# ut-vision/Rot-MVGaze

Hardware: AMD Instinct MI355X
Metric: multi-view samples/sec (fwd+bwd), BxVx3x224x224 (higher is better)
Workload: dtype f32; 1 GPU; C3: ResNet-50, V=4, B=128 per GPU, 3x224x224, fwd+loss+bwd; backbone=ResNet-50, views=4, batch_per_gpu=128, global_batch=128, image=3x224x224, parallelism=dp1, weights=random init, seed 0 (kaiming-normal convs, default Linear), rccl_ranks=1, step_launch=eager: every kernel queued from Python

## Files before the change

include/rotmvgaze.h:

```cpp
#ifndef ROTMVGAZE_H
#define ROTMVGAZE_H

#include <stddef.h>
#include <stdint.h>

#ifdef __cplusplus
extern "C" {
#endif

#define MVG_ABI_VERSION 13

int mvg_abi_version(void);
const char *mvg_last_error(void);
int mvg_device_cus(void);
int mvg_set_scratch(void *ptr, size_t bytes, void *stream);
size_t mvg_scratch_bytes(void);
void *mvg_stream_create_low_priority(void);
int mvg_set_reserved_cus(int n);

enum {
  MVG_K_CONV_FPROP = 0, MVG_K_CONV_DGRAD = 1, MVG_K_CONV_WGRAD = 2, MVG_K_WGRAD_REDUCE = 3,
  MVG_K_BN_FINALIZE = 4, MVG_K_BN_APPLY = 5, MVG_K_BN_BWD_REDUCE = 6, MVG_K_BN_BWD_APPLY = 7,
  MVG_K_POOL = 8, MVG_K_LAYOUT = 9, MVG_K_LINEAR_FPROP = 10, MVG_K_LINEAR_DGRAD = 11,
  MVG_K_LINEAR_WGRAD = 12, MVG_K_ROTCAT = 13, MVG_K_COLSUM = 14, MVG_K_LOSS = 15,
// ... 320 lines not shown
int mvg_bn_apply_split_scaled(const float *y, const float *scale, const float *shift, const void *residual, int residual_sp,
                              const float *res_scale, const float *res_shift, const float *res_sinv, int relu, void *out_sp,
                              const float *out_sinv, uint8_t *relu_bits, int groups, int64_t rows_per_group, int c,
                              void *stream);
int mvg_bn_relu_maxpool_fwd_split_scaled(const float *y, const float *scale, const float *shift, void *pooled_sp,
                                         const float *pooled_sinv, uint8_t *argmax, int groups, int n_per_group, int h, int w,
                                         int c, int ho, int wo, void *stream);
int mvg_avgpool_fwd_split_scaled(const void *x_sp, const float *x_sinv, float *y, int n, int hw, int c, void *stream);
int mvg_conv_dgrad_bn_partials_split(const mvg_conv_desc *d);
int mvg_conv_dgrad_split_bnreduce(const mvg_conv_desc *d, const void *dy_sp, const float *dy_sinv, const void *w_crsk_sp,
                                  const float *w_sinv, float *dx, const float *addend, const float *bn_y, const uint8_t *bn_bits,
                                  const float *bn_mean, const float *bn_invstd, const float *relu_scale, const float *relu_shift,
                                  float *partials, float *s1, float *s2, float *dgamma, float *dbeta, int accumulate,
                                  float *mx, const float *bn_gamma, float *dx_dy_sinv, void *stream);
int mvg_conv_dgrad_split_bnapply_bnreduce(const mvg_conv_desc *d, void *dy_sp, const float *dy_sinv, const float *dz, const float *y,
                                          const float *mean, const float *invstd, const float *gamma, const float *un_s1,
                                          const float *un_s2, int64_t rows_per_group, const void *w_crsk_sp, const float *w_sinv,
                                          float *dx, const float *addend, const float *bn_y, const uint8_t *bn_bits,
                                          const float *bn_mean, const float *bn_invstd, const float *relu_scale,
                                          const float *relu_shift, float *partials, float *s1, float *s2, float *dgamma, float *dbeta,
                                          int accumulate, float *mx, const float *bn_gamma, float *dx_dy_sinv, void *stream);
int mvg_conv_fprop_split_stages(const mvg_conv_desc *d);
int mvg_conv_dgrad_split_stages(const mvg_conv_desc *d, int fused_reduce);
int mvg_conv_fprop_split_bnapply(const mvg_conv_desc *d, void *out_sp, const float *out_sinv, const float *bn_y, const float *scale,
                                 const float *shift, const void *residual, int residual_sp, const float *res_scale,
                                 const float *res_shift, const float *res_sinv, uint8_t *relu_bits, const void *w_sp,
                                 const float *w_sinv, float *y, float *stats, void *stream);
int mvg_stem_rowwindow_split(const float *x_nhwc4, void *xw_sp, int64_t images, int h, int w, void *stream);
int mvg_stem_rowwindow_split_nchw(const float *x_nchw, void *xw_sp, int64_t images, int h, int w, void *stream);
int mvg_stem_fprop_split(const mvg_conv_desc *d, const void *xw_sp, const void *w_sp, const float *w_sinv, float *y, float *stats,
                         void *stream);
int mvg_stem_wgrad_splits_split(const mvg_conv_desc *d);
int mvg_stem_wgrad_split(const mvg_conv_desc *d, const void *xw_sp, const void *dy_sp, const float *dy_sinv, float *dw_rw,
                         float *workspace, int splits, int accumulate, void *stream);
int mvg_bn_relu_maxpool_bwd_reduce_split(const float *g_pooled, const uint8_t *argmax, const float *y, const float *mean,
                                         const float *invstd, const float *scale, const float *shift, int groups,
                                         int n_per_group, int h, int w, int c, int ho, int wo, float *s1, float *s2,
                                         float *dgamma, float *dbeta, int accumulate, float *workspace, float *mx, const float *gamma,
                                         float *dy_sinv, void *stream);
int mvg_bn_relu_maxpool_bwd_apply_split(const float *g_pooled, const uint8_t *argmax, const float *y, const float *mean,
                                        const float *invstd, const float *gamma, const float *scale, const float *shift,
                                        const float *s1, const float *s2, int groups, int n_per_group, int h, int w, int c,
                                        int ho, int wo, void *dy_sp, const float *mx, float *dy_sinv, int dy_sinv_ready, void *stream);
int mvg_conv_wgrad_splits_split(const mvg_conv_desc *d);
int mvg_conv_wgrad_split_tile(const mvg_conv_desc *d, int32_t *bm, int32_t *bn, int32_t *incremental);
int mvg_conv_wgrad_split(const mvg_conv_desc *d, const void *x_sp, const void *dy_sp, const float *dy_sinv, float *dw,
// ... 63 lines not shown
```

rot-mvgaze_amd/_lib.py:

```python
from __future__ import annotations

import ctypes as C
import os

_HERE = os.path.dirname(os.path.abspath(__file__))
LIB_PATH = os.path.join(_HERE, "csrc", "librotmvgaze_hip.so")

K_FAMILIES = 18
ABI_VERSION = 13
SESSION_FP32, SESSION_BF16 = 0, 1


class ConvDesc(C.Structure):
    _fields_ = [(n, C.c_int32) for n in
                ("groups", "n", "h", "w", "cin", "cout", "r", "s", "stride", "pad", "ho", "wo")]

    @classmethod
    def make(cls, groups, n, h, w, cin, cout, k, stride, pad):
        ho = (h + 2 * pad - k) // stride + 1
        wo = (w + 2 * pad - k) // stride + 1
        return cls(groups, n, h, w, cin, cout, k, k, stride, pad, ho, wo)

    @classmethod
    def linear(cls, rows, fin, fout):
# ... 81 lines not shown
    "mvg_bn_apply_split": (_I, [_P, _P, _P, _P, _I, _P, _P, _I, _P, _P, _I, _I64, _I, _P]),
    "mvg_bn_bwd_apply_split": (_I, [_P, _P, _P, _P, _P, _P, _P, _P, _P, _I, _I64, _I, _P, _P, _P, _I, _P]),
    "mvg_bn_bwd_reduce_split": (_I, [_P, _P, _P, _P, _P, _P, _P, _I, _I64, _I, _P, _P, _P, _P, _I, _P, _P, _P, _P, _P, _P]),
    "mvg_bn_relu_maxpool_fwd_split": (_I, [_P, _P, _P, _P, _P, _I, _I, _I, _I, _I, _I, _I, _P]),
    "mvg_avgpool_fwd_split": (_I, [_P, _P, _I, _I, _I, _P]),
    "mvg_act_scales": (_I, [_P, _I, _P, _I, _P]),
    "mvg_bn_apply_split_scaled": (_I, [_P, _P, _P, _P, _I, _P, _P, _P, _I, _P, _P, _P, _I, _I64, _I, _P]),
    "mvg_bn_relu_maxpool_fwd_split_scaled": (_I, [_P, _P, _P, _P, _P, _P, _I, _I, _I, _I, _I, _I, _I, _P]),
    "mvg_avgpool_fwd_split_scaled": (_I, [_P, _P, _P, _I, _I, _I, _P]),
    "mvg_conv_wgrad_split_xs": (_I, [_D, _P, _P, _P, _P, _P, _P, _I, _I, _P]),
    "mvg_conv_wgrad_split_slabs_xs": (_I, [_D, _P, _P, _P, _P, _P, _I, _P]),
    "mvg_stem_rowwindow_split": (_I, [_P, _P, _I64, _I, _I, _P]),
    "mvg_stem_rowwindow_split_nchw": (_I, [_P, _P, _I64, _I, _I, _P]),
    "mvg_stem_fprop_split": (_I, [_D, _P, _P, _P, _P, _P, _P]),
    "mvg_stem_wgrad_splits_split": (_I, [_D]),
    "mvg_stem_wgrad_split": (_I, [_D, _P, _P, _P, _P, _P, _I, _I, _P]),
    "mvg_bn_relu_maxpool_bwd_reduce_split": (_I, [_P, _P, _P, _P, _P, _P, _P, _I, _I, _I, _I, _I, _I, _I, _P, _P, _P, _P, _I, _P, _P, _P, _P, _P]),
    "mvg_bn_relu_maxpool_bwd_apply_split": (_I, [_P, _P, _P, _P, _P, _P, _P, _P, _P, _P, _I, _I, _I, _I, _I, _I, _I, _P, _P, _P, _I, _P]),
    "mvg_conv_dgrad_bn_partials_split": (_I, [_D]),
    "mvg_conv_dgrad_split_bnreduce": (_I, [_D, _P, _P, _P, _P, _P, _P, _P, _P, _P, _P, _P, _P, _P, _P, _P, _P, _P, _I, _P, _P, _P, _P]),
    "mvg_conv_dgrad_split_bnapply_bnreduce": (_I, [_D] + [_P] * 9 + [_I64] + [_P] * 15 + [_I, _P, _P, _P, _P]),
    "mvg_conv_fprop_split_stages": (_I, [_D]),
    "mvg_conv_dgrad_split_stages": (_I, [_D, _I]),
    "mvg_conv_fprop_split_bnapply": (_I, [_D] + [_P] * 6 + [_I] + [_P] * 9),
    "mvg_conv_wgrad_splits_split": (_I, [_D]),
    "mvg_conv_wgrad_split_tile": (_I, [_D, C.POINTER(C.c_int32), C.POINTER(C.c_int32), C.POINTER(C.c_int32)]),
    "mvg_conv_wgrad_split": (_I, [_D, _P, _P, _P, _P, _P, _I, _I, _P]),
    "mvg_conv_wgrad_split_slabs": (_I, [_D, _P, _P, _P, _P, _I, _P]),
    "mvg_wgrad_reduce_batch": (_I, [C.POINTER(C.c_void_p), C.POINTER(C.c_void_p), C.POINTER(C.c_int64), C.POINTER(C.c_int32),
                                    C.POINTER(C.c_int32), _I, _P]),
    "mvg_bn_apply_bits": (_I, [_P, _P, _P, _P, _P, _P, _P, _P, _I, _I64, _I, _P]),
    "mvg_bn_bwd_reduce_bits": (_I, [_P, _P, _P, _P, _P, _I, _I64, _I, _P, _P, _P, _P, _I, _P, _P, _P]),
    "mvg_bn_apply_bits_bf16": (_I, [_P, _P, _P, _P, _P, _P, _P, _P, _I, _I64, _I, _P]),
    "mvg_bn_bwd_reduce_bits_bf16": (_I, [_P, _P, _P, _P, _P, _I, _I64, _I, _P, _P, _P, _P, _I, _P, _P, _P]),
    "mvg_bn_bwd_workspace_floats": (C.c_size_t, [_I, _I64, _I]),
    "mvg_bn_bwd_apply": (_I, [_P, _P, _P, _P, _P, _P, _P, _P, _P, _P, _I, _I64, _I, _P, _P, _P]),
    "mvg_maxpool3x3s2_fwd": (_I, [_P, _P, _P, _I, _I, _I, _I, _I, _I, _P]),
    "mvg_maxpool3x3s2_bwd": (_I, [_P, _P, _P, _I, _I, _I, _I, _I, _I, _P]),
    "mvg_bn_relu_maxpool_fwd": (_I, [_P, _P, _P, _P, _P, _I, _I, _I, _I, _I, _I, _I, _P]),
    "mvg_bn_relu_maxpool_bwd_reduce": (_I, [_P, _P, _P, _P, _P, _P, _P, _I, _I, _I, _I, _I, _I, _I, _P, _P, _P, _P, _I, _P,
                                            _P]),
    "mvg_bn_relu_maxpool_bwd_apply": (_I, [_P, _P, _P, _P, _P, _P, _P, _P, _P, _P, _I, _I, _I, _I, _I, _I, _I, _P, _P]),
    "mvg_bn_eval_bwd": (_I, [_P, _P, _P, _P, _P, _P, _P, _P, _P, _F, _I, _I64, _I, _P, _P, _P, _P, _I, _P, _P]),
    "mvg_bn_eval_bwd_workspace_floats": (C.c_size_t, [_I, _I64, _I]),
    "mvg_bn_relu_maxpool_eval_bwd": (_I, [_P, _P, _P, _P, _P, _P, _P, _P, _F, _I, _I, _I, _I, _I, _I, _I, _P, _P, _P, _I, _P,
                                          _P]),
# ... 114 lines not shown
```

rot-mvgaze_amd/csrc/conv_split.hip:

```cpp
#include "bf16_tile.h"
#include "elem.h"

namespace mvg {

typedef _Float16 f16x8 __attribute__((ext_vector_type(8)));

#define SPLIT_ONE(PA, PB, av, bv, acc)                                                                         \
  _Pragma("unroll") for (int i = 0; i < TM; ++i) _Pragma("unroll") for (int j = 0; j < TN; ++j)                \
      acc[i][j] = __builtin_amdgcn_mfma_f32_32x32x16_f16(av[PA][i], bv[PB][j], acc[i][j], 0, 0, 0);
#define SPLIT_PRODUCTS(av, bv, acc) SPLIT_ONE(0, 1, av, bv, acc) SPLIT_ONE(1, 0, av, bv, acc) SPLIT_ONE(0, 0, av, bv, acc)

constexpr int SP_BM = 128, SP_BK = 32;

__global__ __launch_bounds__(256) void split_f32_kernel(const float4 *__restrict__ x, uint4 *__restrict__ out, long long n8, float scale) {
  const long long stride = (long long)gridDim.x * 256;
  for (long long i = (long long)blockIdx.x * 256 + threadIdx.x; i < n8; i += stride) {
    const float4 lo = x[2 * i], hi = x[2 * i + 1];
    const float v[8] = {lo.x * scale, lo.y * scale, lo.z * scale, lo.w * scale, hi.x * scale, hi.y * scale, hi.z * scale, hi.w * scale};
    uint4 q1, q2;
    split2_chunk(v, q1, q2);
    out[2 * i] = q1;
    out[2 * i + 1] = q2;
  }
}
// ... 308 lines not shown
    if constexpr (AFFINE) {
      unpack8(rv[i], r);
    } else {
      const uint4 r1 = make_uint4(__float_as_uint(rv[i][0].x), __float_as_uint(rv[i][0].y), __float_as_uint(rv[i][0].z), __float_as_uint(rv[i][0].w));
      const uint4 r2 = make_uint4(__float_as_uint(rv[i][1].x), __float_as_uint(rv[i][1].y), __float_as_uint(rv[i][1].z), __float_as_uint(rv[i][1].w));
      merge2_chunk(r1, r2, r);
    }
    mb[i] = bn_apply_chunk(v, sc, sh, true, r, AFFINE, rs, rh, !AFFINE, rsi, true, osc, o);
#pragma unroll
    for (int k = 0; k < 8; ++k) o[k] = ok ? o[k] : 0.f;
  }
  __device__ __forceinline__ void store_extra(int i, unsigned off) {
    if (bits_out) bits_out[off >> 5] = (unsigned short)mb[i];
  }
};

#define MVG_SPLIT_RNG 0
#include "conv_split_igemm.inc"
#undef MVG_SPLIT_RNG
#define MVG_SPLIT_RNG 1
#include "conv_split_igemm.inc"
#undef MVG_SPLIT_RNG

template <int BM, int BN, bool INCR>
__global__ __launch_bounds__(256, BN >= 256 ? 2 : 3) void wgrad_split_kernel(WgradParams p) {
  constexpr int BK = 16, WGM = 2, WGN = 2;
  constexpr int WTM = BM / WGM, WTN = BN / WGN;
  constexpr int TM = WTM / 32, TN = WTN / 32;
  constexpr int LDA = BM + 32, LDB = BN + 32;
  constexpr int MV = BM / 8, NVB = BN / 8;
  constexpr int A_TPR = 256 / BK;
  constexpr int A_CPT = MV / A_TPR > 0 ? MV / A_TPR : 1;
  constexpr int B_CPT = (NVB + A_TPR - 1) / A_TPR;
  constexpr int A_ELEMS = BK * LDA, B_ELEMS = BK * LDB;
  constexpr int STAGE = SP_NP * (A_ELEMS + B_ELEMS);
  __shared__ __attribute__((aligned(16))) unsigned short smem[2 * STAGE];

  const int tid = threadIdx.x;
  const int lane = tid & 63, wave = tid >> 6;
  const int wm = wave / WGN, wn = wave % WGN;
  const int li = lane & 31, lh = lane >> 5;
  const WgradTile t = wgrad_tile_id(p);

  const char *dy = reinterpret_cast<const char *>(p.dy);
  const char *x = reinterpret_cast<const char *>(p.x);
  const __amdgpu_buffer_rsrc_t rs_a = make_rsrc(dy + t.m_begin * p.cout * SP_BYTES, (long long)SP_BYTES * t.m_count * p.cout);
// ... 169 lines not shown
struct SplitPlan { int bm, bn, kt_max; long long tiles; bool pipelined; };
static int split_conv_stages(const SplitPlan &pl) { return (pl.pipelined && pl.bn == 128 && pl.bm == SP_BM) ? 2 : 1; }
static SplitPlan split_plan(int ncols, int taps, long long rows, int groups, bool lin, IgemmClass *cls, int ncls) {
  SplitPlan pl;
  pl.bm = lin ? SP_BM : split_tile_rows(ncols, taps, rows);
  pl.bn = ncols >= 128 ? 128 : 64;
  if (lin && pl.bn == 128 && ncls == 1) {
    const long long t128 = (long long)groups * ceil_div(cls[0].rows_per_group, pl.bm) * ceil_div(ncols, 128);
    if (2 * t128 <= compute_cus()) pl.bn = 64;
  }
  pl.tiles = 0, pl.kt_max = 0;
  for (int i = 0; i < ncls; ++i) {
    IgemmClass &c = cls[i];
    c.mtiles_per_group = ceil_div(c.rows_per_group, pl.bm);
    c.KT = ceil_div(c.ktotal, SP_BK);
    c.tile0 = (int)pl.tiles;
    pl.tiles += (long long)groups * c.mtiles_per_group * ceil_div(ncols, pl.bn);
    pl.kt_max = c.KT > pl.kt_max ? c.KT : pl.kt_max;
  }
  pl.pipelined = pl.tiles <= 2LL * compute_cus() || (pl.tiles <= 4LL * compute_cus() && pl.kt_max >= 48);
  return pl;
}

template <bool DGRAD>
static int launch_igemm_split(IgemmParams &p, hipStream_t st, bool lin, int taps, long long rows, AForm af = A_DMA, bool ranged = false) {
  const SplitPlan pl = split_plan(p.ncols, taps, rows, p.groups, lin, p.cls, p.ncls);
  const int bm = pl.bm, bn = pl.bn;
  const bool pipelined = pl.pipelined;
  p.ntiles = ceil_div(p.ncols, bn);
  p.splits = 1;
  p.sk_tiles = 0;
  p.bn_parts = 0;
  for (int i = 0; i < p.ncls; ++i) {
    IgemmClass &c = p.cls[i];
    c.korder = c.ntaps > 1 ? 1 : 0;
    c.per_div = make_fastdiv((unsigned)(c.ntaps > 0 ? c.ntaps : 1));
    c.unit0 = 0;
    c.part0 = p.bn_parts;
    p.bn_parts += c.mtiles_per_group;
    MVG_REQUIRE((c.ntaps >= 1 || (DGRAD && p.bn_part)) && c.ntaps <= 32 && c.ktotal % SP_BK == 0, "split conv: class shape not covered");
  }
  MVG_REQUIRE(pl.tiles < (1LL << 31), "split conv: grid too large");
  if (pl.tiles <= 0) return 0;
  p.nt_out = (!lin && !(DGRAD && p.cls_step == 2)) ? 1 : 0;
  dim3 grid((unsigned)pl.tiles), block(256);
  if (af != A_DMA) {
    MVG_REQUIRE(!lin && bm == SP_BM && p.ntiles == 1 && p.ncls == 1 && DGRAD == (af == A_DY), "split conv: the operand-forming loaders take one column tile");
    if constexpr (DGRAD) {
      if (bn == 128) hipLaunchKernelGGL((igemm_split16_kernel<128, true, false, 2, 1, A_DY>), grid, block, 0, st, p);
      else hipLaunchKernelGGL((igemm_split16_kernel<64, true, false, 2, 1, A_DY>), grid, block, 0, st, p);
      return check_launch("conv_dgrad_split_bnapply");
    } else {
      if (bn == 128 && af == A_OUT_AFFINE) hipLaunchKernelGGL((igemm_split16_kernel<128, false, false, 2, 1, A_OUT_AFFINE>), grid, block, 0, st, p);
      else if (bn == 128) hipLaunchKernelGGL((igemm_split16_kernel<128, false, false, 2, 1, A_OUT_SP>), grid, block, 0, st, p);
      else if (af == A_OUT_AFFINE) hipLaunchKernelGGL((igemm_split16_kernel<64, false, false, 2, 1, A_OUT_AFFINE>), grid, block, 0, st, p);
      else hipLaunchKernelGGL((igemm_split16_kernel<64, false, false, 2, 1, A_OUT_SP>), grid, block, 0, st, p);
      return check_launch("conv_fprop_split_bnapply");
    }
  }
  if (ranged) {
    MVG_REQUIRE(!DGRAD && !lin && p.out_sp && p.out_absmax, "split conv: the range record goes with a forward that stores sp");
    if constexpr (!DGRAD) {
      if (bm == 256) hipLaunchKernelGGL((igemm_split16_ranged_kernel<64, 4>), grid, block, 0, st, p);
      else if (split_conv_stages(pl) == 2) hipLaunchKernelGGL((igemm_split16_ranged_kernel<128, 2, 2>), grid, block, 0, st, p);
      else if (bn == 128) hipLaunchKernelGGL((igemm_split16_ranged_kernel<128>), grid, block, 0, st, p);
      else hipLaunchKernelGGL((igemm_split16_ranged_kernel<64>), grid, block, 0, st, p);
    }
    return check_launch("conv_fprop_split_ranged");
  }
  if (lin) {
    if (bn == 128 && pipelined) hipLaunchKernelGGL((igemm_split16_kernel<128, DGRAD, true, 2, 2>), grid, block, 0, st, p);
    else if (bn == 128) hipLaunchKernelGGL((igemm_split16_kernel<128, DGRAD, true>), grid, block, 0, st, p);
    else if (pipelined) hipLaunchKernelGGL((igemm_split16_kernel<64, DGRAD, true, 2, 2>), grid, block, 0, st, p);
    else hipLaunchKernelGGL((igemm_split16_kernel<64, DGRAD, true>), grid, block, 0, st, p);
  } else if (bm == 256) hipLaunchKernelGGL((igemm_split16_kernel<64, DGRAD, false, 4>), grid, block, 0, st, p);
  else if (split_conv_stages(pl) == 2) hipLaunchKernelGGL((igemm_split16_kernel<128, DGRAD, false, 2, 2>), grid, block, 0, st, p);
  else if (bn == 128) hipLaunchKernelGGL((igemm_split16_kernel<128, DGRAD>), grid, block, 0, st, p);
  else hipLaunchKernelGGL((igemm_split16_kernel<64, DGRAD>), grid, block, 0, st, p);
  return check_launch(DGRAD ? "conv_dgrad_split" : "conv_fprop_split");
}

}

using namespace mvg;

extern "C" {

int mvg_split_f32(const float *x, void *out_sp, int64_t n, float scale, void *stream) {
  MVG_REQUIRE(x && out_sp && n >= 0 && n % 8 == 0, "split_f32: null argument or n %% 8 != 0");
  MVG_REQUIRE(scale > 0.f, "split_f32: scale must be positive (a power of two keeps the round trip exact)");
  if (n == 0) return 0;
// ... 128 lines not shown
  const double bytes = (double)SP_BYTES * (d->groups * (double)d->n * d->h * d->w * d->cin + (double)d->cout * d->r * d->s * d->cin) +
                       4.0 * d->groups * (double)p.rows_per_group * d->cout +
                       (fap ? 8.0 + 1.0 / 4.0 : 0.0) * d->groups * (double)d->n * d->h * d->w * d->cin;
  const bool lin = d->r == 1 && d->s == 1 && d->h == 1 && d->w == 1;
  ProfScope ps(lin ? MVG_K_LINEAR_FPROP : MVG_K_CONV_FPROP, (hipStream_t)stream, flops, bytes);
  p.stats_partials = ceil_div(p.rows_per_group, SP_BM) * 2;
  return launch_igemm_split<false>(p, (hipStream_t)stream, aff && aff->lin, d->r * d->s, p.rows_per_group,
                                   fap ? (fap->res_scale ? A_OUT_AFFINE : A_OUT_SP) : A_DMA, aff && aff->range_word);
}

int mvg_conv_fprop_split(const mvg_conv_desc *d, const void *x_sp, const float *x_sinv, const void *w_sp, const float *w_sinv, float *y,
                         float *stats, void *stream) {
  return fprop_split_impl(d, x_sp, x_sinv, w_sp, w_sinv, y, stats, stream, nullptr);
}

int mvg_conv_fprop_split_stages(const mvg_conv_desc *d) {
  if (validate_split(d)) return -1;
  IgemmClass c;
  memset(&c, 0, sizeof(c));
  c.rows_per_group = (long long)d->n * d->ho * d->wo;
  c.ktotal = d->r * d->s * d->cin;
  const SplitPlan pl = split_plan(d->cout, d->r * d->s, c.rows_per_group, d->groups, false, &c, 1);
  return split_conv_stages(pl);
}

int mvg_conv_fprop_split_bnapply(const mvg_conv_desc *d, void *out_sp, const float *out_sinv, const float *bn_y, const float *scale,
                                 const float *shift, const void *residual, int residual_sp, const float *res_scale,
                                 const float *res_shift, const float *res_sinv, uint8_t *relu_bits, const void *w_sp,
                                 const float *w_sinv, float *y, float *stats, void *stream) {
  MVG_REQUIRE(d && out_sp && bn_y && scale && shift && residual && w_sp && y, "fprop_split_bnapply: null argument");
  MVG_REQUIRE(d->r == 1 && d->s == 1 && d->stride == 1 && d->pad == 0, "fprop_split_bnapply: 1x1, stride 1, pad 0 only");
  MVG_REQUIRE(d->cout == 64 || d->cout == 128, "fprop_split_bnapply: cout must be 64 or 128 (one column tile; got %d)", d->cout);
  MVG_REQUIRE(d->cin % 32 == 0 && d->cin <= BNA_MAX_C, "fprop_split_bnapply: cin must be a multiple of 32, at most %d (got %d)", BNA_MAX_C,
              d->cin);
  MVG_REQUIRE(residual_sp ? (!res_scale && !res_shift) : (res_scale && res_shift && !res_sinv),
              "fprop_split_bnapply: the residual is an sp identity (no res_scale / res_shift) or fp32 with res_scale and res_shift");
  MVG_REQUIRE((long long)d->n * d->h * d->w * d->cin < (1ll << 29), "fprop_split_bnapply: a group of the input exceeds 2 GiB");
  const SplitFwdApply a = {bn_y, scale, shift, res_scale, res_shift, res_sinv, residual, relu_bits};
  return fprop_split_impl(d, out_sp, out_sinv, w_sp, w_sinv, y, stats, stream, nullptr, -1, -1, &a);
}

int mvg_conv_fprop_split_affine(const mvg_conv_desc *d, const void *x_sp, const float *x_sinv, const void *w_sp, const float *w_sinv,
                                void *out, int out_sp, const float *scale, const float *shift, const void *residual, int residual_sp,
                                int relu, void *stream) {
  MVG_REQUIRE(scale && shift && out, "fprop_split_affine: scale, shift and out are required");
  const SplitAffine a = {scale, shift, residual, residual_sp, relu, out_sp, 0, nullptr, nullptr, nullptr, nullptr};
// ... 64 lines not shown
                       (bnf ? 8.25 : 4.0) * d->groups * (double)d->n * d->h * d->w * d->cin +
                       (bna ? 8.0 : 0.0) * d->groups * (double)d->n * d->ho * d->wo * d->cout;
  const bool lin = d->r == 1 && d->s == 1 && d->h == 1 && d->w == 1;
  ProfScope ps(lin ? MVG_K_LINEAR_DGRAD : MVG_K_CONV_DGRAD, (hipStream_t)stream, flops, bytes);
  if (int e = dgrad_classes(p, d, bnf != nullptr, 4, dx, addend, (hipStream_t)stream)) return e;
  if (p.ncls == 0) return 0;
  return launch_igemm_split<true>(p, (hipStream_t)stream, lin_kernel, d->r * d->s, (long long)d->n * d->h * d->w, bna ? A_DY : A_DMA);
}

int mvg_conv_dgrad_split(const mvg_conv_desc *d, const void *dy_sp, const float *dy_sinv, const void *w_crsk_sp, const float *w_sinv,
                         float *dx, const float *addend, const void *relu_mask_sp, void *stream) {
  MVG_REQUIRE(!relu_mask_sp || d->stride == 1, "dgrad_split: the sp ReLU mask is for stride-1 launches (Linear layers)");
  return dgrad_split_impl(d, dy_sp, dy_sinv, w_crsk_sp, w_sinv, dx, addend, stream, nullptr, relu_mask_sp);
}

int mvg_conv_dgrad_split_stages(const mvg_conv_desc *d, int fused_reduce) {
  if (validate_split(d)) return -1;
  IgemmParams p;
  memset(&p, 0, sizeof(p));
  if (dgrad_geometry(p, d, SP_BYTES, SP_BYTES, "split conv")) return -1;
  DgradDropped dropped;
  dgrad_plan_classes(p, d, fused_reduce != 0, dropped);
  return split_conv_stages(split_plan(p.ncols, d->r * d->s, (long long)d->n * d->h * d->w, p.groups, false, p.cls, p.ncls));
}

int mvg_conv_dgrad_bn_partials_split(const mvg_conv_desc *d) {
  if (validate_split(d)) return -1;
  return dgrad_bn_partials(d, split_tile_rows(d->cin, d->r * d->s, (long long)d->n * d->h * d->w));
}

static int dgrad_split_bnreduce_impl(const char *who, const mvg_conv_desc *d, const void *dy_sp, const float *dy_sinv, const void *w_crsk_sp,
                                     const float *w_sinv, float *dx, const float *addend, const float *bn_y, const uint8_t *bn_bits,
                                     const float *bn_mean, const float *bn_invstd, const float *relu_scale, const float *relu_shift,
                                     float *partials, float *s1, float *s2, float *dgamma, float *dbeta, int accumulate, float *mx,
                                     const float *bn_gamma, float *dx_dy_sinv, void *stream, const SplitBnApply *bna) {
  MVG_REQUIRE(bn_y && bn_mean && bn_invstd && partials && s1 && s2, "%s: null argument", who);
  MVG_REQUIRE((bn_gamma == nullptr) == (dx_dy_sinv == nullptr) && (!dx_dy_sinv || mx), "%s: bn_gamma, dx_dy_sinv (and mx) go together", who);
  MVG_REQUIRE(!(bn_bits && relu_scale) && ((relu_scale == nullptr) == (relu_shift == nullptr)),
              "%s: give the ReLU mask either as bits or as (relu_scale, relu_shift)", who);
  const int P = mvg_conv_dgrad_bn_partials_split(d);
  MVG_REQUIRE(P > 0, "%s: bad descriptor", who);
  const SplitBnFuse f = {bn_y, bn_bits, bn_mean, bn_invstd, relu_scale, relu_shift, partials, mx ? 3 : 2};
  if (dgrad_split_impl(d, dy_sp, dy_sinv, w_crsk_sp, w_sinv, dx, addend, stream, &f, nullptr, false, nullptr, bna)) return 1;
  ProfScope ps(MVG_K_BN_BWD_REDUCE, (hipStream_t)stream, 0.0, 8.0 * d->groups * (double)P * d->cin);
  return bn_bwd_finalize_launch(partials, d->groups, P, d->cin, s1, s2, dgamma, dbeta, accumulate, (hipStream_t)stream, mx, nullptr, nullptr,
                                bn_gamma, bn_invstd, (long long)d->n * d->h * d->w, dx_dy_sinv);
// ... 248 lines not shown
```

rot-mvgaze_amd/csrc/conv_split_igemm.inc:

```
#ifndef MVG_SPLIT_RNG
#error "conv_split_igemm.inc: define MVG_SPLIT_RNG (0 or 1) before including"
#endif

#if MVG_SPLIT_RNG
template <int BN, int WGM = 2, int STAGES = 1>
__global__ __launch_bounds__(256, STAGES == 2 ? 2 : WGM == 4 ? 3 : 4) void igemm_split16_ranged_kernel(IgemmParams p) {
  constexpr bool DGRAD = false, LIN = false;
  constexpr AForm AF = A_DMA;
#else
template <int BN, bool DGRAD, bool LIN = false, int WGM = 2, int STAGES = 1, AForm AF = A_DMA>
__global__ __launch_bounds__(256, STAGES == 2 ? 2 : (DGRAD || WGM == 4 || AF != A_DMA) ? 3 : 4) void igemm_split16_kernel(IgemmParams p) {
#endif
  constexpr int BM = 64 * WGM, WGN = 4 / WGM, NW = 4;
  static_assert(WGM == 2 || (WGM == 4 && BN == 64), "tiles: 128 x BN (2 x 2 waves) or 256 x 64 (4 x 1)");
  static_assert(STAGES == 1 || STAGES == 2, "one LDS stage, or the two-stage pipeline");
  static_assert(AF == A_DMA || (DGRAD == (AF == A_DY) && !LIN && WGM == 2 && STAGES == 1),
                "operand-forming loaders: dy in backward-data, the block output in forward; 128-row tiles, one stage");
  using Former = std::conditional_t<AF == A_DY, DyFormer, OutFormer<AF == A_OUT_AFFINE>>;
  constexpr int WTM = BM / WGM, WTN = BN / WGN;
  constexpr int TM = WTM / 16, TN = WTN / 16;
  constexpr int SLOTS = 4 * SP_NP;
  constexpr int ROWB = 16 * SLOTS, ROWS = BM + BN, STAGE_B = ROWS * ROWB;
  constexpr int NQ = ROWS * SLOTS / 64;
  constexpr int QA = BM * SLOTS / 64;
  constexpr int A_PER = QA / NW, B_PER = (NQ - QA) / NW;
  static_assert(QA % NW == 0 && (NQ - QA) % NW == 0, "whole instructions per wave");
  constexpr int EPI_B = bf16_epilogue_bytes<BM, BN, WGM, DGRAD>();
  constexpr int INFO_OFF = STAGES * STAGE_B > EPI_B ? STAGES * STAGE_B : EPI_B;
  constexpr int BNK_OFF = INFO_OFF + BM * 8;
  constexpr int SMEM_B = BNK_OFF + (AF != A_DMA ? Former::TABLES : 0) * BNA_MAX_C * 4;
  __shared__ __attribute__((aligned(16))) unsigned char smem[SMEM_B];

  const int tid = threadIdx.x;
  const int lane = tid & 63, wave = __builtin_amdgcn_readfirstlane(tid >> 6);
  const int wm = wave / WGN, wn = wave % WGN;
  const int nwg = gridDim.x;
  const int wg_all = p.no_remap ? (int)blockIdx.x : xcd_remap(blockIdx.x, nwg);
  int ci = 0;
  for (int i = 1; i < p.ncls; ++i) ci += wg_all >= p.cls[i].tile0;
  const IgemmClass &c = p.cls[ci];
  const int wg = wg_all - c.tile0;
  const int ntile = wg % p.ntiles;
  const int mt_all = wg / p.ntiles;
  const int g = mt_all / c.mtiles_per_group;
  const int mtile = mt_all - g * c.mtiles_per_group;
  const int KT = c.KT;
  const int ohw = c.out_h * c.out_w;

  uint2 *rowinfo = reinterpret_cast<uint2 *>(smem + INFO_OFF);
  if (tid < BM) {
    const long long m = (long long)mtile * BM + tid;
    const bool ok = m < c.rows_per_group;
    const int mm = ok ? (int)m : 0;
    const int img = (int)fdiv((unsigned)mm, c.ohw_div);
    const int rem = mm - img * ohw;
    const int oy = (int)fdiv((unsigned)rem, c.ow_div), ox = rem - oy * c.out_w;
    const int y0 = DGRAD ? oy + c.cls_cy : oy * p.stride - p.pad;
    const int x0 = DGRAD ? ox + c.cls_cx : ox * p.stride_w - p.pad_w;
    const unsigned base = (unsigned)(img * p.src_img_stride * SP_BYTES) + (unsigned)((y0 * p.src_w + x0) * p.src_c) * (unsigned)SP_BYTES;
    unsigned msk = 0;
    for (int t = 0; t < c.ntaps; ++t) {
      const int fr = (int)fdiv((unsigned)t, c.tap_ns_div), fs = t - fr * c.tap_ns;
      const int iy = DGRAD ? y0 - fr : y0 + fr;
      const int ix = DGRAD ? x0 - fs : x0 + fs;
      msk |= (unsigned)(((unsigned)iy < (unsigned)p.src_h) & ((unsigned)ix < (unsigned)p.src_w)) << t;
    }
    rowinfo[tid] = make_uint2(base, ok ? msk : 0u);
  }
  if constexpr (AF != A_DMA) Former::stage(reinterpret_cast<float *>(smem + BNK_OFF), p, g, p.src_c, tid);
  __syncthreads();
  unsigned a_base[A_PER], a_vmask[A_PER], b_base[B_PER];
#pragma unroll
  for (int i = 0; i < A_PER; ++i) {
    const int sl = (wave + NW * i) * 64 + lane;
    const int row = sl / SLOTS, j = (sl % SLOTS) ^ sp_row_swz(row);
    const uint2 ri = rowinfo[row];
    a_base[i] = ri.x + 16u * (unsigned)j;
    a_vmask[i] = ri.y;
  }
#pragma unroll
  for (int i = 0; i < B_PER; ++i) {
    const int sl = (wave + NW * (A_PER + i)) * 64 + lane - BM * SLOTS;
    const int row = sl / SLOTS, j = (sl % SLOTS) ^ sp_row_swz(row);
    const int n = ntile * BN + row;
    b_base[i] = pred_off(((unsigned)n * (unsigned)p.b_row_len) * (unsigned)SP_BYTES + 16u * (unsigned)j, n < p.ncols);
  }
  const __amdgpu_buffer_rsrc_t rs_a =
      make_rsrc(reinterpret_cast<const char *>(p.a) + (long long)g * p.imgs_per_group * p.src_img_stride * SP_BYTES, p.a_group_bytes);
  const __amdgpu_buffer_rsrc_t rs_b = make_rsrc(p.b, p.b_bytes);
  typedef __attribute__((address_space(3))) void *lds_vp;

  auto issue = [&](int kt, int stage_off) {
    int kstart = kt * SP_BK;
    if (c.korder) {
      const int cblk = (int)fdiv((unsigned)kt, c.per_div), rem = kt - cblk * c.ntaps;
      kstart = (rem << p.src_c_shift) + cblk * SP_BK;
    }
    const int ks = __builtin_amdgcn_readfirstlane(kstart);
    const int tap_u = c.ntaps > 1 ? (ks >> p.src_c_shift) : 0;
    const int chb = ks - (tap_u << p.src_c_shift);
    const int fru = (int)fdiv((unsigned)tap_u, c.tap_ns_div), fsu = tap_u - fru * c.tap_ns;
    const int disp = (fru * p.src_w + fsu) * p.src_c;
    const unsigned sdelta = (unsigned)(((DGRAD ? -disp : disp) + chb) * SP_BYTES);
    unsigned kb = (unsigned)ks * (unsigned)SP_BYTES;
    if (DGRAD) {
      const int btap = (c.tap_r0 + p.tap_step * fru) * p.s + c.tap_s0 + p.tap_step * fsu;
      kb = (unsigned)(btap * p.src_c + chb) * (unsigned)SP_BYTES;
    }
    if constexpr (AF == A_DMA) {
#pragma unroll
      for (int i = 0; i < A_PER; ++i) {
        const bool ok = ((a_vmask[i] >> tap_u) & 1u) != 0u;
        __builtin_amdgcn_raw_ptr_buffer_load_lds(rs_a, (lds_vp)(smem + stage_off + (wave + NW * i) * 1024), 16, (int)pred_off(a_base[i] + sdelta, ok), 0, 0, 0);
      }
    }
#pragma unroll
    for (int i = 0; i < B_PER; ++i)
      __builtin_amdgcn_raw_ptr_buffer_load_lds(rs_b, (lds_vp)(smem + stage_off + (wave + NW * (A_PER + i)) * 1024), 16, (int)(b_base[i] + kb), 0, 0, 0);
  };

  f32x4 acc[TM][TN];
#pragma unroll
  for (int i = 0; i < TM; ++i)
#pragma unroll
    for (int j = 0; j < TN; ++j)
#pragma unroll
      for (int e = 0; e < 4; ++e) acc[i][j][e] = 0.f;

  const int cc_l = lane >> 4;
  int a_off[TM][SP_NP], b_off[TN][SP_NP];
#pragma unroll
  for (int i = 0; i < TM; ++i) {
    const int R = wm * WTM + i * 16 + (lane & 15);
#pragma unroll
    for (int pc = 0; pc < SP_NP; ++pc) a_off[i][pc] = R * ROWB + (((2 * cc_l + pc) ^ sp_row_swz(R)) << 4);
  }
#pragma unroll
  for (int j = 0; j < TN; ++j) {
    const int R = wn * WTN + j * 16 + (lane & 15);
#pragma unroll
    for (int pc = 0; pc < SP_NP; ++pc) b_off[j][pc] = (BM + R) * ROWB + (((2 * cc_l + pc) ^ sp_row_swz(R)) << 4);
  }

  auto load_frags = [&](const unsigned char *stage, f16x8 (&av)[SP_NP][TM], f16x8 (&bv)[SP_NP][TN]) {
#pragma unroll
    for (int pc = 0; pc < SP_NP; ++pc) {
#pragma unroll
      for (int i = 0; i < TM; ++i) av[pc][i] = *reinterpret_cast<const f16x8 *>(stage + a_off[i][pc]);
#pragma unroll
      for (int j = 0; j < TN; ++j) bv[pc][j] = *reinterpret_cast<const f16x8 *>(stage + b_off[j][pc]);
    }
  };
  auto products = [&](const f16x8 (&av)[SP_NP][TM], const f16x8 (&bv)[SP_NP][TN]) { SPLIT16_ONE(0, 1) SPLIT16_ONE(1, 0) SPLIT16_ONE(0, 0) };
  if constexpr (AF != A_DMA) {
    const int C = p.src_c;
    const int a_cc = tid & 3, a_r0 = tid >> 2;
    const long long grow0 = (long long)g * c.rows_per_group;
    Former f(p, grow0, c.rows_per_group, C);
    uint4 *a_out = reinterpret_cast<uint4 *>(const_cast<float *>(p.a)) + grow0 * C / 4;
    bool a_ok[2];
    unsigned a_goff[2];
#pragma unroll
    for (int i = 0; i < 2; ++i) {
      const long long m = (long long)mtile * BM + a_r0 + 64 * i;
      a_ok[i] = m < c.rows_per_group;
      a_goff[i] = pred_off((unsigned)m * (unsigned)C * 4u + 32u * (unsigned)a_cc, a_ok[i]);
    }
    auto a_load = [&](int kt) {
#pragma unroll
      for (int i = 0; i < 2; ++i) f.load(i, a_goff[i] + 128u * (unsigned)kt);
    };
    constexpr bool PREFETCH = BN == 64;
    if (PREFETCH) a_load(0);
    for (int kt = 0; kt < KT; ++kt) {
      issue(kt, 0);
      if (!PREFETCH) a_load(kt);
// ... 47 lines not shown
      issue(1, STAGE_B);
      asm volatile("s_waitcnt vmcnt(%0)\n\ts_barrier" ::"n"(G) : "memory");
    } else {
      asm volatile("s_waitcnt vmcnt(0)\n\ts_barrier" ::: "memory");
    }
    f16x8 a0[SP_NP][TM], b0[SP_NP][TN], a1[SP_NP][TM], b1[SP_NP][TN];
    load_frags(smem, a0, b0);
    int cur = 0;
    auto step = [&](int kt, const f16x8 (&ca)[SP_NP][TM], const f16x8 (&cb)[SP_NP][TN], f16x8 (&na)[SP_NP][TM], f16x8 (&nb)[SP_NP][TN]) {
      if (kt + 1 < KT) {
        asm volatile("s_waitcnt vmcnt(0) lgkmcnt(0)\n\ts_barrier" ::: "memory");
        if (kt + 2 < KT) issue(kt + 2, cur);
        cur ^= STAGE_B;
        load_frags(smem + cur, na, nb);
      }
      products(ca, cb);
    };
    for (int kt = 0; kt < KT; kt += 2) {
      step(kt, a0, b0, a1, b1);
      if (kt + 1 < KT) step(kt + 1, a1, b1, a0, b0);
    }
    __syncthreads();
  }
#if MVG_SPLIT_RNG
  bf16_epilogue<BM, BN, WGM, DGRAD, true, WGM, true, DGRAD, LIN, WGN, false, true>(p, c, acc, reinterpret_cast<unsigned short *>(smem), tid, g, mtile,
                                                                                     ntile);
#else
  bf16_epilogue<BM, BN, WGM, DGRAD, true, WGM, true, DGRAD, LIN, WGN>(p, c, acc, reinterpret_cast<unsigned short *>(smem), tid, g, mtile, ntile);
#endif
}
```

rot-mvgaze_amd/ops.py:

```python
from __future__ import annotations

import ctypes as C
from typing import Optional

import torch

from ._lib import ConvDesc, K_FAMILIES, ProfEntry, check, lib

Tensor = torch.Tensor


def _p(t: Optional[Tensor]):
    if t is None:
        return None
    assert t.is_cuda and t.dtype in _PTR_DTYPES, (t.device, t.dtype)
    return t.data_ptr()


_PTR_DTYPES = frozenset((torch.float32, torch.int32, torch.uint8, torch.int16, torch.bfloat16, torch.float16))
_workspaces = {}
_MAX_WORKSPACES = 8
_raw_stream = getattr(torch._C, "_cuda_getCurrentRawStream", None)


# ... 211 lines not shown
    if n < 0:
        check(1, "conv_stats_partials_split")
    return n, rpp.value


def conv_fprop_split(d: ConvDesc, x_sp: Tensor, w_sp: Tensor, y: Tensor, stats: Optional[Tensor] = None):
    check(lib().mvg_conv_fprop_split(C.byref(d), _p(x_sp), _sinv(x_sp), _p(w_sp), _sinv(w_sp), _p(y), _p(stats), _s()), "conv_fprop_split")


def conv_fprop_split_stages(d: ConvDesc) -> int:
    n = lib().mvg_conv_fprop_split_stages(C.byref(d))
    if n < 0:
        check(1, "conv_fprop_split_stages")
    return n


def conv_dgrad_split_stages(d: ConvDesc, fused_reduce: bool = False) -> int:
    n = lib().mvg_conv_dgrad_split_stages(C.byref(d), int(fused_reduce))
    if n < 0:
        check(1, "conv_dgrad_split_stages")
    return n


def conv_wgrad_split_tile(d: ConvDesc):
    bm, bn, incr = C.c_int32(0), C.c_int32(0), C.c_int32(0)
    if lib().mvg_conv_wgrad_split_tile(C.byref(d), C.byref(bm), C.byref(bn), C.byref(incr)) != 0:
        check(1, "conv_wgrad_split_tile")
    return bm.value, bn.value, bool(incr.value)


def conv_fprop_split_bnapply(d: ConvDesc, out_sp: Tensor, bn_y, scale, shift, residual, w_sp: Tensor, y: Tensor,
                             stats: Optional[Tensor] = None, residual_affine=None, bits: Optional[Tensor] = None):
    assert bits is None or (bits.dtype == torch.uint8 and bits.numel() == d.groups * d.n * d.h * d.w * d.cin // 4)
    rs, rh = residual_affine if residual_affine is not None else (None, None)
    res_sp = is_sp(residual)
    check(lib().mvg_conv_fprop_split_bnapply(C.byref(d), _p(out_sp), _sinv(out_sp), _p(bn_y), _p(scale), _p(shift), _p(residual), int(res_sp),
                                             _p(rs), _p(rh), _sinv(residual) if res_sp else None, _p(bits), _p(w_sp), _sinv(w_sp), _p(y),
                                             _p(stats), _s()), "conv_fprop_split_bnapply")


def conv_fprop_split_affine(d: ConvDesc, x_sp: Tensor, w_sp: Tensor, out: Tensor, scale: Tensor, shift: Tensor,
                            residual: Optional[Tensor], relu: bool):
    assert getattr(residual, "sinv", None) is None, "conv_fprop_split_affine: the residual is read unscaled"
    check(lib().mvg_conv_fprop_split_affine(C.byref(d), _p(x_sp), _sinv(x_sp), _p(w_sp), _sinv(w_sp), _p(out), int(is_sp(out)), _p(scale),
                                            _p(shift), _p(residual), int(is_sp(residual)), int(relu), _s()), "conv_fprop_split_affine")

# ... 543 lines not shown
```

Baseline: 1690 samples/s.

## Add halo-tile loader for 3x3 stride-1 split implicit-GEMM convolutions

Adds a new implicit-GEMM kernel variant for 3x3 stride-1 pad-1 convolutions. It loads one contiguous halo window of input pixel rows into LDS per channel block and reuses it across all nine taps by shifting the row offset, instead of issuing a fresh A-tile gather per tap. Out-of-image taps are zeroed with per-row tap masks. A selection rule enables it by default only for certain dgrad shapes (bm=128/bn=128 with src_c>=128, and bm=256 with src_c=64 on large grids). A runtime mode switch and query functions are also exposed. This trades larger LDS use and possibly lower occupancy for fewer global loads.

```diff
diff --git a/include/rotmvgaze.h b/include/rotmvgaze.h
--- a/include/rotmvgaze.h
+++ b/include/rotmvgaze.h
@@ -366,6 +366,9 @@
                                           int accumulate, float *mx, const float *bn_gamma, float *dx_dy_sinv, void *stream);
 int mvg_conv_fprop_split_stages(const mvg_conv_desc *d);
 int mvg_conv_dgrad_split_stages(const mvg_conv_desc *d, int fused_reduce);
+int mvg_set_split_halo(int mode);
+int mvg_conv_fprop_split_loader(const mvg_conv_desc *d);
+int mvg_conv_dgrad_split_loader(const mvg_conv_desc *d, int fused_reduce);
 int mvg_conv_fprop_split_bnapply(const mvg_conv_desc *d, void *out_sp, const float *out_sinv, const float *bn_y, const float *scale,
                                  const float *shift, const void *residual, int residual_sp, const float *res_scale,
                                  const float *res_shift, const float *res_sinv, uint8_t *relu_bits, const void *w_sp,
diff --git a/rot-mvgaze_amd/_lib.py b/rot-mvgaze_amd/_lib.py
--- a/rot-mvgaze_amd/_lib.py
+++ b/rot-mvgaze_amd/_lib.py
@@ -127,6 +127,9 @@
     "mvg_conv_dgrad_split_bnapply_bnreduce": (_I, [_D] + [_P] * 9 + [_I64] + [_P] * 15 + [_I, _P, _P, _P, _P]),
     "mvg_conv_fprop_split_stages": (_I, [_D]),
     "mvg_conv_dgrad_split_stages": (_I, [_D, _I]),
+    "mvg_set_split_halo": (_I, [_I]),
+    "mvg_conv_fprop_split_loader": (_I, [_D]),
+    "mvg_conv_dgrad_split_loader": (_I, [_D, _I]),
     "mvg_conv_fprop_split_bnapply": (_I, [_D] + [_P] * 6 + [_I] + [_P] * 9),
     "mvg_conv_wgrad_splits_split": (_I, [_D]),
     "mvg_conv_wgrad_split_tile": (_I, [_D, C.POINTER(C.c_int32), C.POINTER(C.c_int32), C.POINTER(C.c_int32)]),
diff --git a/rot-mvgaze_amd/csrc/conv_split.hip b/rot-mvgaze_amd/csrc/conv_split.hip
--- a/rot-mvgaze_amd/csrc/conv_split.hip
+++ b/rot-mvgaze_amd/csrc/conv_split.hip
@@ -354,6 +354,15 @@
 #include "conv_split_igemm.inc"
 #undef MVG_SPLIT_RNG
 
+constexpr int split_halo_lds(int bn, int halo, int nbuf) { return (halo + nbuf * bn) * 128; }
+constexpr int split_halo_wgs(int bn, int halo, int nbuf) {
+  const int n = 160 * 1024 / (split_halo_lds(bn, halo, nbuf) + 4096);
+  return n > 3 ? 3 : n;
+}
+#define MVG_SPLIT_RNG 2
+#include "conv_split_igemm.inc"
+#undef MVG_SPLIT_RNG
+
 template <int BM, int BN, bool INCR>
 __global__ __launch_bounds__(256, BN >= 256 ? 2 : 3) void wgrad_split_kernel(WgradParams p) {
   constexpr int BK = 16, WGM = 2, WGN = 2;
@@ -569,6 +578,34 @@
   return pl;
 }
 
+static int split_halo_rows(const SplitPlan &pl, const IgemmParams &p, bool dgrad, bool lin, AForm af, bool ranged) {
+  if (lin || af != A_DMA || ranged || p.ncls != 1 || split_conv_stages(pl) != 1) return 0;
+  if (p.r != 3 || p.s != 3 || p.stride != 1 || p.pad != 1 || p.cls[0].ntaps != 9) return 0;
+  if (dgrad ? p.cls_step != 1 : (p.stride_w != 1 || p.pad_w != 1)) return 0;
+  if (p.src_h != p.cls[0].out_h || p.src_w != p.cls[0].out_w || p.src_img_stride != (long long)p.src_h * p.src_w * p.src_c) return 0;
+  const int span = pl.bm + 2 * p.src_w + 2;
+  if (pl.bm == 256) return span <= 384 ? 384 : 0;
+  return span <= 192 ? 192 : (span <= 256 ? 256 : 0);
+}
+#ifndef MVG_HALO_NBUF_256
+#define MVG_HALO_NBUF_256 2
+#endif
+#ifndef MVG_HALO_NBUF_128
+#define MVG_HALO_NBUF_128 1
+#endif
+static int g_split_halo = 1;
+static bool split_halo_admits(const SplitPlan &pl, int halo, int src_c, bool dgrad, bool bnreduce) {
+  if (pl.bm == SP_BM && pl.bn == 128 && halo == 192) return dgrad && src_c >= 128;
+  if (pl.bm == 256) return dgrad && !bnreduce && src_c == 64 && pl.tiles >= 16LL * compute_cus();
+  return false;
+}
+static int split_loader_halo(const SplitPlan &pl, const IgemmParams &p, bool dgrad, bool bnreduce, bool lin, AForm af, bool ranged) {
+  if (g_split_halo == 0) return 0;
+  const int halo = split_halo_rows(pl, p, dgrad, lin, af, ranged);
+  if (halo == 0 || g_split_halo == 2) return halo;
+  return split_halo_admits(pl, halo, p.src_c, dgrad, bnreduce) ? halo : 0;
+}
+
 template <bool DGRAD>
 static int launch_igemm_split(IgemmParams &p, hipStream_t st, bool lin, int taps, long long rows, AForm af = A_DMA, bool ranged = false) {
   const SplitPlan pl = split_plan(p.ncols, taps, rows, p.groups, lin, p.cls, p.ncls);
@@ -614,6 +651,14 @@
       else hipLaunchKernelGGL((igemm_split16_ranged_kernel<64>), grid, block, 0, st, p);
     }
     return check_launch("conv_fprop_split_ranged");
+  }
+  if (const int halo = split_loader_halo(pl, p, DGRAD, p.bn_part != nullptr, lin, af, ranged)) {
+    if (bm == 256) hipLaunchKernelGGL((igemm_split16_halo_kernel<64, DGRAD, 4, 384, MVG_HALO_NBUF_256>), grid, block, 0, st, p);
+    else if (bn == 128 && halo == 192) hipLaunchKernelGGL((igemm_split16_halo_kernel<128, DGRAD, 2, 192, MVG_HALO_NBUF_128>), grid, block, 0, st, p);
+    else if (bn == 128) hipLaunchKernelGGL((igemm_split16_halo_kernel<128, DGRAD, 2, 256, MVG_HALO_NBUF_128>), grid, block, 0, st, p);
+    else if (halo == 192) hipLaunchKernelGGL((igemm_split16_halo_kernel<64, DGRAD, 2, 192, MVG_HALO_NBUF_128>), grid, block, 0, st, p);
+    else hipLaunchKernelGGL((igemm_split16_halo_kernel<64, DGRAD, 2, 256, MVG_HALO_NBUF_128>), grid, block, 0, st, p);
+    return check_launch(DGRAD ? "conv_dgrad_split(halo)" : "conv_fprop_split(halo)");
   }
   if (lin) {
     if (bn == 128 && pipelined) hipLaunchKernelGGL((igemm_split16_kernel<128, DGRAD, true, 2, 2>), grid, block, 0, st, p);
@@ -788,6 +833,22 @@
   c.ktotal = d->r * d->s * d->cin;
   const SplitPlan pl = split_plan(d->cout, d->r * d->s, c.rows_per_group, d->groups, false, &c, 1);
   return split_conv_stages(pl);
+}
+
+int mvg_set_split_halo(int mode) {
+  MVG_REQUIRE(mode >= 0 && mode <= 2, "set_split_halo: mode must be 0 (never), 1 (the shipped rule) or 2 (wherever eligible), got %d", mode);
+  g_split_halo = mode;
+  return 0;
+}
+
+int mvg_conv_fprop_split_loader(const mvg_conv_desc *d) {
+  if (validate_split(d)) return -1;
+  IgemmParams p;
+  memset(&p, 0, sizeof(p));
+  if (fprop_geometry(p, d, SP_BYTES, SP_BYTES, "split conv")) return -1;
+  const bool lin = d->r == 1 && d->s == 1 && d->h == 1 && d->w == 1;
+  const SplitPlan pl = split_plan(p.ncols, d->r * d->s, p.rows_per_group, p.groups, false, p.cls, p.ncls);
+  return split_loader_halo(pl, p, false, false, lin, A_DMA, false) ? 1 : 0;
 }
 
 int mvg_conv_fprop_split_bnapply(const mvg_conv_desc *d, void *out_sp, const float *out_sinv, const float *bn_y, const float *scale,
@@ -898,6 +959,19 @@
   DgradDropped dropped;
   dgrad_plan_classes(p, d, fused_reduce != 0, dropped);
   return split_conv_stages(split_plan(p.ncols, d->r * d->s, (long long)d->n * d->h * d->w, p.groups, false, p.cls, p.ncls));
+}
+
+int mvg_conv_dgrad_split_loader(const mvg_conv_desc *d, int fused_reduce) {
+  if (validate_split(d)) return -1;
+  IgemmParams p;
+  memset(&p, 0, sizeof(p));
+  if (dgrad_geometry(p, d, SP_BYTES, SP_BYTES, "split conv")) return -1;
+  DgradDropped dropped;
+  dgrad_plan_classes(p, d, fused_reduce != 0, dropped);
+  if (p.ncls == 0) return 0;
+  const bool lin = d->r == 1 && d->s == 1 && d->h == 1 && d->w == 1;
+  const SplitPlan pl = split_plan(p.ncols, d->r * d->s, (long long)d->n * d->h * d->w, p.groups, false, p.cls, p.ncls);
+  return split_loader_halo(pl, p, true, fused_reduce != 0, lin, A_DMA, false) ? 1 : 0;
 }
 
 int mvg_conv_dgrad_bn_partials_split(const mvg_conv_desc *d) {
diff --git a/rot-mvgaze_amd/csrc/conv_split_igemm.inc b/rot-mvgaze_amd/csrc/conv_split_igemm.inc
--- a/rot-mvgaze_amd/csrc/conv_split_igemm.inc
+++ b/rot-mvgaze_amd/csrc/conv_split_igemm.inc
@@ -1,8 +1,15 @@
 #ifndef MVG_SPLIT_RNG
-#error "conv_split_igemm.inc: define MVG_SPLIT_RNG (0 or 1) before including"
-#endif
-
-#if MVG_SPLIT_RNG
+#error "conv_split_igemm.inc: define MVG_SPLIT_RNG (0, 1 or 2) before including"
+#endif
+
+#if MVG_SPLIT_RNG == 2
+template <int BN, bool DGRAD, int WGM, int HALO, int NBUF>
+__global__ __launch_bounds__(256, split_halo_wgs(BN, HALO, NBUF)) void igemm_split16_halo_kernel(IgemmParams p) {
+  constexpr bool LIN = false;
+  constexpr AForm AF = A_DMA;
+  constexpr int STAGES = 1;
+  static_assert(HALO % 32 == 0 && HALO >= 64 * WGM + 4 && (NBUF == 1 || NBUF == 2), "halo rows: whole instructions per wave");
+#elif MVG_SPLIT_RNG == 1
 template <int BN, int WGM = 2, int STAGES = 1>
 __global__ __launch_bounds__(256, STAGES == 2 ? 2 : WGM == 4 ? 3 : 4) void igemm_split16_ranged_kernel(IgemmParams p) {
   constexpr bool DGRAD = false, LIN = false;
@@ -26,7 +33,15 @@
   constexpr int A_PER = QA / NW, B_PER = (NQ - QA) / NW;
   static_assert(QA % NW == 0 && (NQ - QA) % NW == 0, "whole instructions per wave");
   constexpr int EPI_B = bf16_epilogue_bytes<BM, BN, WGM, DGRAD>();
+#if MVG_SPLIT_RNG == 2
+  constexpr int B_ROW0 = HALO, B_B = BN * ROWB;
+  constexpr int LOAD_B = (HALO + NBUF * BN) * ROWB;
+  static_assert(LOAD_B == split_halo_lds(BN, HALO, NBUF), "the launch bound's LDS bytes");
+  constexpr int INFO_OFF = LOAD_B > EPI_B ? LOAD_B : EPI_B;
+#else
+  constexpr int B_ROW0 = BM;
   constexpr int INFO_OFF = STAGES * STAGE_B > EPI_B ? STAGES * STAGE_B : EPI_B;
+#endif
   constexpr int BNK_OFF = INFO_OFF + BM * 8;
   constexpr int SMEM_B = BNK_OFF + (AF != A_DMA ? Former::TABLES : 0) * BNA_MAX_C * 4;
   __shared__ __attribute__((aligned(16))) unsigned char smem[SMEM_B];
@@ -69,7 +84,9 @@
   }
   if constexpr (AF != A_DMA) Former::stage(reinterpret_cast<float *>(smem + BNK_OFF), p, g, p.src_c, tid);
   __syncthreads();
-  unsigned a_base[A_PER], a_vmask[A_PER], b_base[B_PER];
+  unsigned b_base[B_PER];
+#if MVG_SPLIT_RNG != 2
+  unsigned a_base[A_PER], a_vmask[A_PER];
 #pragma unroll
   for (int i = 0; i < A_PER; ++i) {
     const int sl = (wave + NW * i) * 64 + lane;
@@ -78,6 +95,7 @@
     a_base[i] = ri.x + 16u * (unsigned)j;
     a_vmask[i] = ri.y;
   }
+#endif
 #pragma unroll
   for (int i = 0; i < B_PER; ++i) {
     const int sl = (wave + NW * (A_PER + i)) * 64 + lane - BM * SLOTS;
@@ -90,6 +108,29 @@
   const __amdgpu_buffer_rsrc_t rs_b = make_rsrc(p.b, p.b_bytes);
   typedef __attribute__((address_space(3))) void *lds_vp;
 
+#if MVG_SPLIT_RNG == 2
+  constexpr int HQ = HALO / (8 * NW);
+  const int src_w = p.src_w;
+  const int hrows = BM + 2 * src_w + 2;
+  const unsigned h_rowb = (unsigned)p.src_c * (unsigned)SP_BYTES;
+  const int h_row0 = wave * 8 + (lane >> 3);
+  const int h_pix0 = mtile * BM - src_w - 1 + h_row0;
+  const unsigned h_base = (unsigned)h_pix0 * h_rowb + 16u * (unsigned)((lane & 7) ^ sp_row_swz(h_row0));
+  auto issue_halo = [&](int cblk) {
+    const unsigned cb = (unsigned)(cblk * SP_BK * SP_BYTES);
+#pragma unroll
+    for (int i = 0; i < HQ; ++i)
+      if ((wave + NW * i) * 8 < hrows)
+        __builtin_amdgcn_raw_ptr_buffer_load_lds(rs_a, (lds_vp)(smem + (wave + NW * i) * 1024), 16,
+                                                 (int)pred_off(h_base + (unsigned)(8 * NW * i) * h_rowb + cb, h_pix0 + 8 * NW * i >= 0), 0, 0, 0);
+  };
+  auto issue_b = [&](int tap, int cblk, int buf) {
+    const unsigned kb = (unsigned)((tap << p.src_c_shift) + cblk * SP_BK) * (unsigned)SP_BYTES;
+#pragma unroll
+    for (int i = 0; i < B_PER; ++i)
+      __builtin_amdgcn_raw_ptr_buffer_load_lds(rs_b, (lds_vp)(smem + (B_ROW0 + buf * BN) * ROWB + (wave + NW * i) * 1024), 16, (int)(b_base[i] + kb), 0, 0, 0);
+  };
+#else
   auto issue = [&](int kt, int stage_off) {
     int kstart = kt * SP_BK;
     if (c.korder) {
@@ -118,6 +159,7 @@
     for (int i = 0; i < B_PER; ++i)
       __builtin_amdgcn_raw_ptr_buffer_load_lds(rs_b, (lds_vp)(smem + stage_off + (wave + NW * (A_PER + i)) * 1024), 16, (int)(b_base[i] + kb), 0, 0, 0);
   };
+#endif
 
   f32x4 acc[TM][TN];
 #pragma unroll
@@ -128,20 +170,52 @@
       for (int e = 0; e < 4; ++e) acc[i][j][e] = 0.f;
 
   const int cc_l = lane >> 4;
-  int a_off[TM][SP_NP], b_off[TN][SP_NP];
+  int b_off[TN][SP_NP];
+#if MVG_SPLIT_RNG != 2
+  int a_off[TM][SP_NP];
 #pragma unroll
   for (int i = 0; i < TM; ++i) {
     const int R = wm * WTM + i * 16 + (lane & 15);
 #pragma unroll
     for (int pc = 0; pc < SP_NP; ++pc) a_off[i][pc] = R * ROWB + (((2 * cc_l + pc) ^ sp_row_swz(R)) << 4);
   }
+#endif
 #pragma unroll
   for (int j = 0; j < TN; ++j) {
     const int R = wn * WTN + j * 16 + (lane & 15);
 #pragma unroll
-    for (int pc = 0; pc < SP_NP; ++pc) b_off[j][pc] = (BM + R) * ROWB + (((2 * cc_l + pc) ^ sp_row_swz(R)) << 4);
-  }
-
+    for (int pc = 0; pc < SP_NP; ++pc) b_off[j][pc] = (B_ROW0 + R) * ROWB + (((2 * cc_l + pc) ^ sp_row_swz(R)) << 4);
+  }
+
+#if MVG_SPLIT_RNG == 2
+  unsigned a_tmask[TM];
+#pragma unroll
+  for (int i = 0; i < TM; ++i) a_tmask[i] = rowinfo[wm * WTM + i * 16 + (lane & 15)].y;
+  auto tap_shift = [&](int tap) {
+    const int fru = (int)fdiv((unsigned)tap, c.tap_ns_div), fsu = tap - fru * c.tap_ns;
+    return DGRAD ? (2 - fru) * src_w + 2 - fsu : fru * src_w + fsu;
+  };
+  auto load_frags = [&](int tap, int buf, f16x8 (&av)[SP_NP][TM], f16x8 (&bv)[SP_NP][TN]) {
+    const int h0 = wm * WTM + (lane & 15) + tap_shift(tap);
+#pragma unroll
+    for (int pc = 0; pc < SP_NP; ++pc) {
+      const unsigned char *src = smem + h0 * ROWB + (((2 * cc_l + pc) ^ sp_row_swz(h0)) << 4);
+#pragma unroll
+      for (int i = 0; i < TM; ++i) av[pc][i] = *reinterpret_cast<const f16x8 *>(src + i * 16 * ROWB);
+#pragma unroll
+      for (int j = 0; j < TN; ++j) bv[pc][j] = *reinterpret_cast<const f16x8 *>(smem + buf * B_B + b_off[j][pc]);
+    }
+  };
+  auto mask_frags = [&](int tap, f16x8 (&av)[SP_NP][TM]) {
+    const f16x8 zero = {0, 0, 0, 0, 0, 0, 0, 0};
+#pragma unroll
+    for (int i = 0; i < TM; ++i) {
+      const bool ok = ((a_tmask[i] >> tap) & 1u) != 0u;
+#pragma unroll
+      for (int pc = 0; pc < SP_NP; ++pc) av[pc][i] = ok ? av[pc][i] : zero;
+    }
+  };
+#else
   auto load_frags = [&](const unsigned char *stage, f16x8 (&av)[SP_NP][TM], f16x8 (&bv)[SP_NP][TN]) {
 #pragma unroll
     for (int pc = 0; pc < SP_NP; ++pc) {
@@ -151,7 +225,68 @@
       for (int j = 0; j < TN; ++j) bv[pc][j] = *reinterpret_cast<const f16x8 *>(stage + b_off[j][pc]);
     }
   };
+#endif
   auto products = [&](const f16x8 (&av)[SP_NP][TM], const f16x8 (&bv)[SP_NP][TN]) { SPLIT16_ONE(0, 1) SPLIT16_ONE(1, 0) SPLIT16_ONE(0, 0) };
+#if MVG_SPLIT_RNG == 2
+  auto next_tap = [&](int &tap, int &cblk) {
+    if (++tap == c.ntaps) tap = 0, ++cblk;
+  };
+  if constexpr (NBUF == 1) {
+    int tap = 0, cblk = 0;
+    for (int kt = 0; kt < KT; ++kt) {
+      if (tap == 0) issue_halo(cblk);
+      issue_b(tap, cblk, 0);
+      asm volatile("s_waitcnt vmcnt(0)\n\ts_barrier" ::: "memory");
+      {
+        f16x8 av[SP_NP][TM], bv[SP_NP][TN];
+        load_frags(tap, 0, av, bv);
+        mask_frags(tap, av);
+        products(av, bv);
+      }
+      asm volatile("s_waitcnt lgkmcnt(0)\n\ts_barrier" ::: "memory");
+      next_tap(tap, cblk);
+    }
+  } else {
+    f16x8 a0[SP_NP][TM], b0[SP_NP][TN], a1[SP_NP][TM], b1[SP_NP][TN];
+    int tap = 0, cblk = 0;
+    issue_halo(0);
+    issue_b(0, 0, 0);
+    asm volatile("s_waitcnt vmcnt(0)\n\ts_barrier" ::: "memory");
+    if (KT > 1) {
+      int t1 = 0, c1 = 0;
+      next_tap(t1, c1);
+      issue_b(t1, c1, 1);
+    }
+    load_frags(0, 0, a0, b0);
+    auto step = [&](int kt, f16x8 (&ca)[SP_NP][TM], const f16x8 (&cb)[SP_NP][TN], f16x8 (&na)[SP_NP][TM], f16x8 (&nb)[SP_NP][TN]) {
+      int t1 = tap, c1 = cblk;
+      next_tap(t1, c1);
+      const bool more = kt + 1 < KT, opens = more && t1 == 0;
+      if (more) {
+        asm volatile("s_waitcnt vmcnt(0) lgkmcnt(0)\n\ts_barrier" ::: "memory");
+        if (opens) issue_halo(c1);
+        if (kt + 2 < KT) {
+          int t2 = t1, c2 = c1;
+          next_tap(t2, c2);
+          issue_b(t2, c2, kt & 1);
+        }
+        if (!opens) load_frags(t1, (kt + 1) & 1, na, nb);
+      }
+      mask_frags(tap, ca);
+      products(ca, cb);
+      if (opens) {
+        asm volatile("s_waitcnt vmcnt(0)\n\ts_barrier" ::: "memory");
+        load_frags(t1, (kt + 1) & 1, na, nb);
+      }
+      tap = t1, cblk = c1;
+    };
+    for (int kt = 0; kt < KT; kt += 2) {
+      step(kt, a0, b0, a1, b1);
+      if (kt + 1 < KT) step(kt + 1, a1, b1, a0, b0);
+    }
+    asm volatile("s_waitcnt lgkmcnt(0)\n\ts_barrier" ::: "memory");
+  }
+#else
   if constexpr (AF != A_DMA) {
     const int C = p.src_c;
     const int a_cc = tid & 3, a_r0 = tid >> 2;
@@ -245,7 +380,8 @@
     }
     __syncthreads();
   }
-#if MVG_SPLIT_RNG
+#endif
+#if MVG_SPLIT_RNG == 1
   bf16_epilogue<BM, BN, WGM, DGRAD, true, WGM, true, DGRAD, LIN, WGN, false, true>(p, c, acc, reinterpret_cast<unsigned short *>(smem), tid, g, mtile,
                                                                                      ntile);
 #else
diff --git a/rot-mvgaze_amd/ops.py b/rot-mvgaze_amd/ops.py
--- a/rot-mvgaze_amd/ops.py
+++ b/rot-mvgaze_amd/ops.py
@@ -257,6 +257,24 @@
     return n
 
 
+def set_split_halo(mode: int):
+    check(lib().mvg_set_split_halo(int(mode)), "set_split_halo")
+
+
+def conv_fprop_split_loader(d: ConvDesc) -> int:
+    n = lib().mvg_conv_fprop_split_loader(C.byref(d))
+    if n < 0:
+        check(1, "conv_fprop_split_loader")
+    return n
+
+
+def conv_dgrad_split_loader(d: ConvDesc, fused_reduce: bool = False) -> int:
+    n = lib().mvg_conv_dgrad_split_loader(C.byref(d), int(fused_reduce))
+    if n < 0:
+        check(1, "conv_dgrad_split_loader")
+    return n
+
+
 def conv_wgrad_split_tile(d: ConvDesc):
     bm, bn, incr = C.c_int32(0), C.c_int32(0), C.c_int32(0)
     if lib().mvg_conv_wgrad_split_tile(C.byref(d), C.byref(bm), C.byref(bn), C.byref(incr)) != 0:
```

Result: no change. 1685 samples/s (-0.3%).
